# johannes-graeter/limo

Hardware: AMD Instinct MI355X
Metric: keyframe-BA window solves/sec (5 KF, ~2k landmarks) (higher is better)
Workload: dtype f64; 1 GPU; C2: KITTI-00-shaped windows, 5 keyframes x 2000 landmarks, LiDAR depth + ground plane, solveTrimmed schedule {2, trim 5%, <=100 LM iterations}; batch_windows_per_gpu=16384, distinct_windows_per_gpu=4096, observations_per_batch=144288124, depth_observations_per_batch=68405568, parallelism=single, converged=16328

## Files before the change

### limo_amd/csrc/kba_batch_plan.hpp

```cpp
#pragma once
#include <algorithm>
#include <cstdint>
#include <vector>

#include "kba_items.hpp"
#include "kba_pack.hpp"

namespace kba {

struct PlanKernelSizes {
    int (*lean_lds)(int ncol);
    int (*wide_lds)(int nfp, int nc, int n_view);
    int lin_lds;
    int wide_waves;
    int trim_max_sort;
};

struct BatchPlan {
    bool any_fast = false, any_gen = false;
    int plain_tm = 1, plain_wpe = 4, gp_tm = 1, gp_wpe = 3;
    bool pair_ok = false;
    int wide_npw = 0;
    int plain_lds = 0, leangp_lds = 0, wide_lds = 0;
    int max_nc = 0;
    int asm_bytes = 0, solve_bytes = 0, trim_bytes = 0;
    int schur_wave_lds = 0;
    int onelaunch_lds = 0;
};

inline BatchPlan plan_batch(const PackedBatch& P, const PlanKernelSizes& ks) {
    BatchPlan p;
    int t_gen = 1, nfp_gen = 16, nc_gen = kCamSlots, nv_gen = 1, max_nfq = 0, max_nf = 0;
    for (const WinDesc& d : P.win) {
        p.max_nc = std::max(p.max_nc, (int)d.nc);
        if (d.schur_fast) {
            p.any_fast = true;
            max_nfq = std::max(max_nfq, (int)d.nfq);
            max_nf = std::max(max_nf, (int)d.nf);
        } else if (d.n_sblk > 0) {
            p.any_gen = true;
            t_gen = std::max(t_gen, d.nf_pad / 16);
            nfp_gen = std::max(nfp_gen, (int)d.nf_pad);
            nc_gen = std::max(nc_gen, (int)d.nc);
            nv_gen = std::max(nv_gen, (int)d.n_view);
        }
    }
    if (p.any_fast) {
        p.plain_tm = (max_nfq + 16) / 16 <= 1 ? 1 : 2;
        p.plain_wpe = p.plain_tm == 1 ? 4 : 3;
        p.plain_lds = ks.lean_lds(max_nfq + 1);
        p.gp_tm = std::min(3, (max_nf + 16) / 16);
        p.gp_wpe = p.gp_tm == 1 ? 3 : 2;
        p.leangp_lds = ks.lean_lds(max_nf + 1);
        p.pair_ok = p.plain_tm == 2 && p.gp_tm == 3;
    }
    if (p.any_gen) {
        const int tiles = t_gen * (t_gen + 1) / 2, npw = (tiles + ks.wide_waves - 1) / ks.wide_waves;
        p.wide_npw = npw <= 1 ? 1 : npw <= 3 ? 3 : npw <= 6 ? 6 : npw <= 12 ? 12 : -1;
        p.wide_lds = ks.wide_lds(nfp_gen, nc_gen, nv_gen);
    }
    {
        int nc_lds = kCamSlots, nf_lds = 1, nv_lds = 1;
        for (const WinDesc& d : P.win)
            if (d.cam_scr_off < 0) {
                nc_lds = std::max(nc_lds, (int)d.nc);
                nf_lds = std::max(nf_lds, (int)d.nf);
                nv_lds = std::max(nv_lds, (int)d.n_view);
            }
        p.asm_bytes = cam_assemble_scratch(nc_lds, kBlock, nv_lds) * (int)sizeof(double);
        p.solve_bytes = cam_solve_scratch(nc_lds, kBlock, nf_lds) * (int)sizeof(double);
    }
    int max_lm = 1, np2 = 1;
    for (const WinDesc& d : P.win) max_lm = std::max(max_lm, (int)d.n_lm);
    while (np2 < max_lm) np2 <<= 1;
    p.trim_bytes = np2 <= ks.trim_max_sort ? np2 * 12 + max_lm + 16 : 16;
    p.schur_wave_lds = (std::max(p.plain_lds, p.leangp_lds) + 15) / 16 * 16;
    p.onelaunch_lds = std::max(std::max(p.asm_bytes, p.solve_bytes), std::max(p.trim_bytes, ks.lin_lds));
    return p;
}

inline void build_sblk_list(const PackedBatch& P, const std::vector<int32_t>* windows, int span, int span_gp, int owner, std::vector<int32_t>& v,
                            int& n_plain, int& n_fgp) {
    v.clear();
    n_plain = n_fgp = 0;
    const int nw = windows ? (int)windows->size() : P.n_win;
    for (int cls = 0; cls < 3; ++cls) {
        for (int q = 0; q < nw; ++q) {
            const int w = windows ? (*windows)[q] : q;
            const WinDesc& d = P.win[w];
// ... 15 lines not shown
```

### limo_amd/csrc/kba_kernels.hip

```cpp
#include <hip/hip_runtime.h>

#include <type_traits>

#define KBA_SYNC() __syncthreads()
#include "kba_items.hpp"

namespace kba {

__device__ __forceinline__ double wave_sum(double v) {
#pragma unroll
    for (int off = 32; off > 0; off >>= 1) v += __shfl_down(v, off, 64);
    return v;
}
__device__ __forceinline__ double wave_max(double v) {
#pragma unroll
    for (int off = 32; off > 0; off >>= 1) v = fmax(v, __shfl_down(v, off, 64));
    return v;
}

template <int N>
__device__ __forceinline__ void block_sum(const double* vals, double* lds , double* out_global) {
    const int lane = threadIdx.x & 63, wave = threadIdx.x >> 6;
#pragma unroll
    for (int i = 0; i < N; ++i) {
        const double s = wave_sum(vals[i]);
        if (lane == 0) lds[wave * N + i] = s;
    }
    __syncthreads();
    if (threadIdx.x < N) {
        out_global[threadIdx.x] = (lds[threadIdx.x] + lds[N + threadIdx.x]) + (lds[2 * N + threadIdx.x] + lds[3 * N + threadIdx.x]);
    }
}

__device__ __forceinline__ double dpp_mov(double x, int ctrl_sel) {
    int lo = __double2loint(x), hi = __double2hiint(x);
    switch (ctrl_sel) {
        case 0:
            lo = __builtin_amdgcn_update_dpp(0, lo, 0x128, 0xF, 0xF, false);
            hi = __builtin_amdgcn_update_dpp(0, hi, 0x128, 0xF, 0xF, false);
            break;
        case 1:
            lo = __builtin_amdgcn_update_dpp(0, lo, 0x141, 0xF, 0xF, false);
            hi = __builtin_amdgcn_update_dpp(0, hi, 0x141, 0xF, 0xF, false);
            break;
        case 2:
            lo = __builtin_amdgcn_update_dpp(0, lo, 0x4E, 0xF, 0xF, false);
            hi = __builtin_amdgcn_update_dpp(0, hi, 0x4E, 0xF, 0xF, false);
            break;
        default:
            lo = __builtin_amdgcn_update_dpp(0, lo, 0xB1, 0xF, 0xF, false);
            hi = __builtin_amdgcn_update_dpp(0, hi, 0xB1, 0xF, 0xF, false);
            break;
    }
    return __hiloint2double(hi, lo);
}
__device__ __forceinline__ double swap32_add(double a, double b) {
    auto lo = __builtin_amdgcn_permlane32_swap((unsigned)__double2loint(a), (unsigned)__double2loint(b), false, false);
    auto hi = __builtin_amdgcn_permlane32_swap((unsigned)__double2hiint(a), (unsigned)__double2hiint(b), false, false);
    return __hiloint2double((int)hi[0], (int)lo[0]) + __hiloint2double((int)hi[1], (int)lo[1]);
}
__device__ __forceinline__ double swap16_add(double a, double b) {
    auto lo = __builtin_amdgcn_permlane16_swap((unsigned)__double2loint(a), (unsigned)__double2loint(b), false, false);
    auto hi = __builtin_amdgcn_permlane16_swap((unsigned)__double2hiint(a), (unsigned)__double2hiint(b), false, false);
    return __hiloint2double((int)hi[0], (int)lo[0]) + __hiloint2double((int)hi[1], (int)lo[1]);
}
template <int CTRL>
__device__ __forceinline__ double halve_dpp(double a, double b, bool bit) {
    const double keep = bit ? b : a, send = bit ? a : b;
    return keep + dpp_mov(send, CTRL);
}
__device__ __forceinline__ double wave_sum_all(double v) {
    v = swap32_add(v, v);
    v = swap16_add(v, v);
    v += dpp_mov(v, 0);
    v += dpp_mov(v, 1);
    v += dpp_mov(v, 2);
    return v + dpp_mov(v, 3);
}
__device__ __forceinline__ int rs28_index(int lane) {
    const int row = lane >> 4, b3 = (lane >> 3) & 1, b2 = (lane >> 2) & 1, b1 = (lane >> 1) & 1;
    int j;
    if (!b1 && !b2) j = b3 ? 4 : 0;
    else if (!b1 && b2) j = b3 ? 6 : 2;
    else if (b1 && !b2) j = b3 ? 5 : 1;
    else j = b3 ? -1 : 3;
    return (lane & 1) || j < 0 ? -1 : 7 * row + j;
}
__device__ __forceinline__ double wave_reduce_scatter28(const double* v, int lane) {
    double s[14], u[7];
#pragma unroll
    for (int i = 0; i < 14; ++i) s[i] = swap32_add(v[i], v[i + 14]);
#pragma unroll
    for (int i = 0; i < 7; ++i) u[i] = swap16_add(s[i], s[i + 7]);
    const bool b3 = lane & 8, b2 = lane & 4, b1 = lane & 2;
    const double w0 = halve_dpp<0>(u[0], u[4], b3), w1 = halve_dpp<0>(u[1], u[5], b3), w2 = halve_dpp<0>(u[2], u[6], b3);
    const double w3 = u[3] + dpp_mov(u[3], 0);
    const double x0 = halve_dpp<1>(w0, w2, b2), x1 = halve_dpp<1>(w1, w3, b2);
    const double y = halve_dpp<2>(x0, x1, b1);
    return y + dpp_mov(y, 3);
}
__device__ __forceinline__ int rs14_index(int lane) {
    const int half = lane >> 5, rowp = (lane >> 4) & 1, b3 = (lane >> 3) & 1, b2 = (lane >> 2) & 1;
    const int j = b2 ? (b3 ? 3 : 1) : (b3 ? 2 : 0);
    if ((lane & 3) || (j == 3 && rowp)) return -1;
    return 7 * half + (j == 3 ? 3 : j + 4 * rowp);
}
__device__ __forceinline__ double wave_reduce_scatter14(const double* v, int lane) {
    double s[7];
#pragma unroll
    for (int i = 0; i < 7; ++i) s[i] = swap32_add(v[i], v[i + 7]);
    const double u0 = swap16_add(s[0], s[4]), u1 = swap16_add(s[1], s[5]), u2 = swap16_add(s[2], s[6]);
    const double u3 = swap16_add(s[3], s[3]);
    const bool b3 = lane & 8, b2 = lane & 4;
    const double w0 = halve_dpp<0>(u0, u2, b3), w1 = halve_dpp<0>(u1, u3, b3);
    const double x = halve_dpp<1>(w0, w1, b2);
    const double y = x + dpp_mov(x, 2);
    return y + dpp_mov(y, 3);
}
__device__ __forceinline__ void block_sum28(const double* vals, double* lds, double* out_global) {
    const int lane = threadIdx.x & 63, wave = threadIdx.x >> 6;
    const double tot = wave_reduce_scatter28(vals, lane);
    const int idx = rs28_index(lane);
    if (idx >= 0) lds[wave * 28 + idx] = tot;
    __syncthreads();
    if (threadIdx.x < 28) out_global[threadIdx.x] = (lds[threadIdx.x] + lds[28 + threadIdx.x]) + (lds[56 + threadIdx.x] + lds[84 + threadIdx.x]);
}

__device__ __forceinline__ int wl_at(const BatchView& bv, const int32_t* wl, int i) {
    if (bv.counted) return i < wl[-1] ? wl[i] : -1;
    return wl ? wl[i] : i;
}

__global__ void k_solve_init(BatchView bv, SolveConsts c, int max_iter, int select) {
    const int w = blockIdx.x * blockDim.x + threadIdx.x;
    if (w >= bv.n_win) return;
    WinState& s = bv.st[w];
    bool sel = true;
    if (select >= 1) sel = bv.win[w].do_trim != 0;
    if (select == 2) sel = sel && (s.solve_initial_cost - s.solve_final_cost <= 0.0);
    lm_solve_init(s, sel, max_iter, c);
}

__global__ void k_export_active(BatchView bv, int32_t* flags) {
    const int w = blockIdx.x * blockDim.x + threadIdx.x;
    if (w < bv.n_win) flags[w] = bv.st[w].active;
}

__global__ void k_expire(BatchView bv) {
    const int w = blockIdx.x * blockDim.x + threadIdx.x;
    if (w >= bv.n_win) return;
    if (bv.st[w].active) lm_terminate(bv.st[w], LIMO_NO_CONVERGENCE);
}

constexpr int kSchedThreads = 1024;
constexpr int kSchedSlotsPerLane = 4;
constexpr int kSchedMaxSlots = kSchedThreads * kSchedSlotsPerLane;

__global__ void k_sched_advance(BatchView bv, SolveConsts c) {
    const int s = blockIdx.x * blockDim.x + threadIdx.x;
    if (s >= bv.n_slots) return;
    int32_t* cnt = bv.slot_cnt + (int64_t)s * (SL_COUNT + 1);
#pragma unroll
    for (int k = 0; k <= SL_COUNT; ++k) cnt[k] = 0;
    const bool pending = *(volatile int32_t*)bv.sched_ctl < bv.n_win;
    int w = bv.slot_win[s];
    const int w_in = w;
    int kind = 0, n_fin = 0;
    for (int tries = 0; tries < 2; ++tries) {
        if (w < 0) {
            if (!pending) break;
            const int nxt = atomicAdd(bv.sched_ctl, 1);
            if (nxt >= bv.n_win) break;
            w = nxt;
            bv.st[w].phase = PH_IDLE;
        }
        const int r = sched_advance(bv.st[w], bv.win[w], c);
        if (r == 2) {
            ++n_fin;
            w = -1;
            continue;
        }
        kind = r == 1 ? (bv.st[w].phase == PH_TRIM ? 2 : 1) : 0;
        break;
    }
    if (n_fin) atomicAdd(bv.sched_ctl + 1, n_fin);
    if (w != w_in) bv.slot_win[s] = w;
    if (w < 0 || !kind) return;
    const WinDesc& wd = bv.win[w];
    cnt[SL_COUNT] = kind;
    if (kind == 2) {
        cnt[SL_TBLK] = wd.n_blk;
        cnt[SL_TLBLK] = wd.n_lblk;
        cnt[SL_TWIN] = 1;
        return;
    }
    const int gp_groups = (wd.n_sblk - wd.n_sblk_plain + c.schur_span_gp - 1) / c.schur_span_gp;
    const int pl_groups = (wd.n_sblk_plain + c.schur_span - 1) / c.schur_span;
    cnt[SL_LBLK] = wd.n_lblk;
    if (wd.schur_fast) {
        cnt[SL_SPLAIN] = pl_groups;
        cnt[SL_SFGP] = gp_groups;
    } else {
        cnt[SL_SGEN] = pl_groups + gp_groups;
    }
    cnt[SL_WIN] = 1;
}

__global__ __launch_bounds__(kSchedThreads) void k_sched_scan(BatchView bv, int round) {
    __shared__ int wave_tot[16][SL_COUNT];
    const int t = threadIdx.x, lane = t & 63, wave = t >> 6;
    int cnt[kSchedSlotsPerLane][SL_COUNT], tot[SL_COUNT];
#pragma unroll
    for (int k = 0; k < SL_COUNT; ++k) tot[k] = 0;
#pragma unroll
    for (int q = 0; q < kSchedSlotsPerLane; ++q) {
        const int s = t * kSchedSlotsPerLane + q;
#pragma unroll
        for (int k = 0; k < SL_COUNT; ++k) {
            cnt[q][k] = s < bv.n_slots ? bv.slot_cnt[(int64_t)s * (SL_COUNT + 1) + k] : 0;
            tot[k] += cnt[q][k];
        }
    }
    int off[SL_COUNT];
#pragma unroll
    for (int k = 0; k < SL_COUNT; ++k) {
        int x = tot[k];
#pragma unroll
        for (int d = 1; d < 64; d <<= 1) {
            const int y = __shfl_up(x, d, 64);
            if (lane >= d) x += y;
        }
        off[k] = x - tot[k];
        if (lane == 63) wave_tot[wave][k] = x;
    }
    __syncthreads();
    if (t < SL_COUNT) {
        int run = 0;
        for (int q = 0; q < 16; ++q) {
            const int v = wave_tot[q][t];
            wave_tot[q][t] = run;
            run += v;
        }
        bv.sched_lists[bv.sched_off[t]] = run;
    }
    __syncthreads();
#pragma unroll
    for (int q = 0; q < kSchedSlotsPerLane; ++q) {
        const int s = t * kSchedSlotsPerLane + q;
        if (s >= bv.n_slots) continue;
#pragma unroll
        for (int k = 0; k < SL_COUNT; ++k) {
            bv.slot_cnt[(int64_t)s * (SL_COUNT + 1) + k] = wave_tot[wave][k] + off[k];
            off[k] += cnt[q][k];
        }
    }
    if (t == 0) {
        const int done = bv.sched_ctl[1];
        *(volatile int32_t*)(bv.sched_done_host + (round & 3)) = done;
        __threadfence_system();
    }
}

__global__ __launch_bounds__(256) void k_sched_fill(BatchView bv, SolveConsts c) {
    const int s = blockIdx.x * 4 + (threadIdx.x >> 6), lane = threadIdx.x & 63;
    if (s >= bv.n_slots) return;
    const int32_t* off = bv.slot_cnt + (int64_t)s * (SL_COUNT + 1);
    const int kind = off[SL_COUNT];
    if (!kind) return;
    const int w = bv.slot_win[s];
    const WinDesc& wd = bv.win[w];
    auto L = [&](int k) { return bv.sched_lists + bv.sched_off[k] + 1 + off[k]; };
    if (kind == 2) {
        for (int i = lane; i < wd.n_blk; i += 64) L(SL_TBLK)[i] = wd.blk0 + i;
        for (int i = lane; i < wd.n_lblk; i += 64) L(SL_TLBLK)[i] = wd.lblk0 + i;
        if (lane == 0) L(SL_TWIN)[0] = w;
        return;
    }
    for (int i = lane; i < wd.n_lblk; i += 64) L(SL_LBLK)[i] = wd.lblk0 + i;
    const int n_pg = (wd.n_sblk_plain + c.schur_span - 1) / c.schur_span;
    const int n_gg = (wd.n_sblk - wd.n_sblk_plain + c.schur_span_gp - 1) / c.schur_span_gp;
    int32_t* lp = wd.schur_fast ? L(SL_SPLAIN) : L(SL_SGEN);
    int32_t* lg = wd.schur_fast ? L(SL_SFGP) : L(SL_SGEN) + n_pg;
    for (int i = lane; i < n_pg; i += 64) lp[i] = wd.sblk0 + i * c.schur_span;
    for (int i = lane; i < n_gg; i += 64) lg[i] = wd.sblk0 + wd.n_sblk_plain + i * c.schur_span_gp;
    if (lane == 0) L(SL_WIN)[0] = w;
    const WinState& st = bv.st[w];
    if (st.active && st.need_lin && lane < wd.n_view) view_consts_item(bv, wd.view0 + lane);
}

__global__ void k_view_consts(BatchView bv) {
    const int v = blockIdx.x * blockDim.x + threadIdx.x;
    if (v >= bv.TV) return;
    const WinState& st = bv.st[bv.view_win[v]];
    if (!st.active || !st.need_lin) return;
    view_consts_item(bv, v);
}

typedef const double __attribute__((address_space(4))) cdouble;
constexpr int kLinAccl = 13;
constexpr int kLinVlds = 38;
template <bool VLDS>
__device__ __forceinline__ void lin_lm_block(const BatchView& bv, const SolveConsts& c, int b) {
    const int w = bv.lblk_win[b];
    const WinState& st = bv.st[w];
    if (!st.active || !st.need_lin) return;
    const bool want_cost = st.first != 0;
    const WinDesc& wd = bv.win[w];
    const int n_view = wd.n_view;
    const int n = bv.lblk_n[b];
    const int lane = threadIdx.x & 63, wave = threadIdx.x >> 6;
    const bool in_block = (int)threadIdx.x < n;
    const int gl = bv.lblk_lm0[b] + (in_block ? (int)threadIdx.x : n - 1);
    const int state = in_block ? bv.lm_state[gl] : 0;
    LinIn in;
    const bool take_candidate = st.accept != 0;
    const double* lm_src = take_candidate ? bv.lm_c : bv.lm;
    in.p[0] = lm_src[3 * (int64_t)gl];
    in.p[1] = lm_src[3 * (int64_t)gl + 1];
    in.p[2] = lm_src[3 * (int64_t)gl + 2];
    if (take_candidate && in_block) {
        bv.lm[3 * (int64_t)gl] = in.p[0];
        bv.lm[3 * (int64_t)gl + 1] = in.p[1];
        bv.lm[3 * (int64_t)gl + 2] = in.p[2];
    }
    in.w = bv.lm_weight[gl];
    in.sw = sqrt(in.w);
    LmTailIn tail;
    lin_lm_tail_fetch(bv, w, gl, tail);
    const int32_t* slot = bv.lm_slot + gl;
    double* out = bv.lv_part + wd.lvpart_off + (int64_t)(b - wd.lblk0) * n_view * kLinPartial;
    extern __shared__ __attribute__((aligned(16))) double lin_lds[];
    double* const vlds = lin_lds + kLinAccl * kBlock;
    double* const lv_lds = vlds + (VLDS ? n_view * kLinVlds : 0);
    double* const accl = lin_lds + threadIdx.x;
    typedef typename std::conditional<VLDS, const double*, cdouble*>::type VT;
    constexpr int kVStride = VLDS ? kLinVlds : kViewLin;
    VT vc;
    if constexpr (VLDS) {
        const double* src = bv.view_lin + (int64_t)kViewLin * wd.view0;
        for (int i = threadIdx.x; i < n_view * kLinVlds; i += kBlock) vlds[i] = src[(i / kLinVlds) * kViewLin + i % kLinVlds];
        __syncthreads();
        vc = vlds;
    } else {
        vc = (VT)(bv.view_lin + (int64_t)kViewLin * wd.view0);
    }
    const int64_t dump = bv.SO - kObsBlock + threadIdx.x;
#pragma unroll
    for (int i = 0; i < 9; ++i) accl[i * kBlock] = 0.0;
#pragma unroll
    for (int i = 0; i < 3; ++i) accl[(9 + i) * kBlock] = tail.sc[i];
    accl[12 * kBlock] = __hiloint2double(tail.gg, 0);
    auto accum = [&](auto vl, const double* r3, const double* c4) {
        LmAcc a;
#pragma unroll
// ... 1503 lines not shown
```

### limo_amd/csrc/kba_layout.hpp

```cpp
#pragma once
#include <stddef.h>
#include <stdint.h>

#include "../../include/limo_hip.h"

namespace kba {

constexpr int kMaxKf = 20;
constexpr int kMaxViews = 64;
constexpr int kViewLin = 64;
constexpr int kCamSlots = 10;
constexpr int kMaxNc = kMaxKf * kCamSlots;
constexpr int kBlock = 256;
constexpr int kObsPerLane = 4;
constexpr int kObsBlock = kBlock * kObsPerLane;
constexpr int kSchurLm = 16;
constexpr int kSchurLmPerBlock = 64;
constexpr int kSchurSpan = 2, kSchurSpanGp = 1;
constexpr int kMaxRegRows = 1 + (kMaxKf - 1) * 5 + 3 * kMaxKf;

constexpr int kGpRed = 65;
constexpr int kLinPartial = 28;
constexpr int kLinWaves = 4;

// ... 102 lines not shown
    int32_t slab_packed;
};

struct BatchView {
    int32_t n_win, TK, TL, TO, TV, TG, n_blk, n_lblk, n_sblk, Vmax;
    int64_t SO, SL, SG;
    const WinDesc* win;
    WinState* st;
    WinRed* red;
    double *pose, *pdir, *pdist, *lm;
    double *pose_c, *pdir_c, *pdist_c, *lm_c;
    const int32_t* kf_win;
    const int32_t* kf_blk0;
    const int32_t* kf_nblk;
    const int32_t* kf_gp0;
    const int32_t* kf_ngp;
    uint8_t* cmask;
    uint8_t* cpresent;
    const int32_t* cslot;
    const int32_t* lm_win;
    const int32_t* lm_id;
    const double* lm_weight;
    uint8_t* lm_state;
    const int32_t* lm_gp;
    const int32_t* lm_slot;
    const int32_t* view_kf;
    const int32_t* view_win;
    const double* view_cam;
    double* view_lin_c;
    double* view_lin;
    const int32_t* blk_view;
    const int32_t* blk_obs0;
    const int32_t* blk_n;
    const int32_t* obs_lm;
    const float *obs_u, *obs_v, *obs_d;
    const int32_t* lblk_win;
    const int32_t* lblk_lm0;
    const int32_t* lblk_n;
    const int32_t* sblk_win;
    const int32_t* sblk_lm0;
    const int32_t* sblk_n;
    const SchurGroup* sgrp;
    const int32_t* lblk_owner;
    const int32_t* gp_owner;
    double* x_lv;
    double* x_lf;
    double* x_gp;
    double* x_gc;
    double* x_gcc;
    double* x_lb;
    const double* gp_red;
    int32_t gp_red_P, pad_x;
    const int32_t* gp_lm;
    const int32_t* gp_kf;
    const double* gp_w;
    double *gp_r, *gp_F, *gp_E;
    double* gp_cost;
    double* gp_cost_c;
    double *obs_r, *obs_c;
    double *obs_Jp, *obs_Jl;
    const EvalChunk* echunk;
    int64_t SD;
    int32_t n_echunk, pad_e;
    double* lv_part;
    double* lblk_linfail;
    double *lm_V, *lm_g;
    double *lm_scale;
    double* lm_Li;
    double* lblk_part;
    double *Hcc, *gc;
    double *scale_c, *yc, *delta_c;
    double *S_part;
    double *S_red;
    double* cam_scratch;
    double* reg_cost;
    double *trim_rep, *trim_dep;
    int32_t* n_active;
    int32_t* n_active_host;
    int32_t counted;
    int32_t n_slots;
    int32_t* slot_win;
    int32_t* sched_ctl;
    int32_t* slot_cnt;
    int32_t* sched_lists;
    int32_t sched_off[SL_COUNT];
    int32_t* sched_done_host;
};

struct ExchangeLayout {
    int P = 1, n_win = 0, TK = 0;
    size_t n_lv = 0, n_w = 0, n_gp = 0, n_lb = 0, n_S = 0;
    size_t b_lv = 0, b_lf = 0, b_gp = 0, b_gc = 0, b_gcc = 0, b_lb = 0, b_S = 0, b_total = 0;
    size_t c_lv = 0, c_lf = 0, c_gp = 0, c_gc = 0, c_gcc = 0, c_lb = 0, c_S = 0, c_total = 0;
    size_t trim_count = 0;
    size_t spart_count = 1;
#if defined(__HIPCC__)
    __host__ __device__
#endif
    void range(int point, size_t& off, size_t& count) const {
        off = point == 2 ? b_S : point == 4 ? b_gcc : 0;
        const size_t end = point == 1 || point == 4 ? b_S : b_total;
        count = end - off;
    }
};

}
```

### limo_amd/csrc/limo_hip.hip

```cpp
#include <hip/hip_runtime.h>
#include <rccl/rccl.h>

#include <algorithm>
#include <chrono>
#include <cmath>
#include <cstdio>
#include <cstring>
#include <atomic>
#include <memory>
#include <new>
#include <string>
#include <thread>
#include <vector>

#include "kba_kernels.hip"

#include "kba_batch_plan.hpp"
#include "kba_buffers.hpp"
#include "kba_rows.hpp"

using namespace kba;

#include "limo_ctx.hpp"

// ... 545 lines not shown
    }

    void step() override {
        hipStream_t s = ctx->stream;
        if (c.slab_packed) spart_has_packed = true;
        const WorkLists& a = wl[0].cur;
        for (size_t i = 0; i < pv.size(); ++i)
            if (wl[i].cur.n_lblk) {
                hipLaunchKernelGGL(k_lm_damp, dim3(wl[i].cur.n_lblk), dim3(kBlock), 0, s, pv[i], c, wl[i].cur.lblk);
                LAUNCH_CHECK("k_lm_damp");
            }
        {
            EventPair* ep = timed(LIMO_KERNEL_SCHUR);
            for (size_t i = 0; i < pv.size(); ++i) {
                const WorkLists& l = wl[i].cur;
                launch_schur(pv[i], l.sblk, l.n_sblk_plain, l.sblk + l.n_sblk_plain, l.n_sblk_fgp, l.sblk + l.n_sblk_plain + l.n_sblk_fgp,
                             l.n_sblk - l.n_sblk_plain - l.n_sblk_fgp, false, s);
                LAUNCH_CHECK("Schur kernels");
            }
            if (ep) note(hipEventRecord(ep->b, s), "hipEventRecord");
        }
        if (shard_P > 1) {
            if (a.n_win)
                for (size_t i = 0; i < pv.size(); ++i) {
                    hipLaunchKernelGGL(k_shard_reduce, dim3(a.n_win), dim3(kBlock), 0, s, pv[i], a.win, local_shards[i], 1);
                    hipLaunchKernelGGL(k_slab_reduce, dim3(a.n_win, 8), dim3(kBlock), 0, s, pv[i], a.win, shard_P);
                    LAUNCH_CHECK("k_slab_reduce");
                }
            if (assemble_pending) {
                assemble_pending = false;
                exchange(3);
                assemble(it_no - 1);
            } else {
                exchange(2);
            }
        }
        if (a.n_win) hipLaunchKernelGGL(k_cam_solve, dim3(a.n_win), dim3(kBlock), plan.solve_bytes, s, bv, c, a.win);
        LAUNCH_CHECK("k_cam_solve");
        for (size_t i = 0; i < pv.size(); ++i) {
            if (wl[i].cur.n_lblk) {
                hipLaunchKernelGGL(k_backsub, dim3(wl[i].cur.n_lblk), dim3(kBlock), 0, s, pv[i], c, wl[i].cur.lblk);
                LAUNCH_CHECK("k_backsub");
            }
        }
        if (shard_P > 1 && a.n_win)
            for (size_t i = 0; i < pv.size(); ++i) {
                hipLaunchKernelGGL(k_shard_reduce, dim3(a.n_win), dim3(kBlock), 0, s, pv[i], a.win, local_shards[i], 2);
                LAUNCH_CHECK("k_shard_reduce");
            }
        exchange(4);
        if (a.n_win) hipLaunchKernelGGL(k_step_decide, dim3(a.n_win), dim3(64), 0, s, bv, c, a.win);
        LAUNCH_CHECK("k_step_decide");
        hipLaunchKernelGGL(k_accept, dim3(cdiv((int64_t)P.TK + P.TL, 256)), dim3(256), 0, s, bv);
        LAUNCH_CHECK("k_accept");
    }

    void trim() override {
        hipStream_t s = ctx->stream;
        bool any = false;
        for (const WinDesc& d : P.win) any = any || d.do_trim;
        if (!any) return;
        for (size_t i = 0; i < pv.size(); ++i) {
            if (wl[i].full.n_blk) {
                hipLaunchKernelGGL(k_trim_residual, dim3(wl[i].full.n_blk), dim3(kBlock), 0, s, pv[i], d_plane_rep, d_plane_dep, wl[i].full.blk);
                LAUNCH_CHECK("k_trim_residual");
            }
        }
        if (P.TL) {
            for (size_t i = 0; i < pv.size(); ++i) {
                hipLaunchKernelGGL(k_trim_max, dim3(cdiv(P.TL, 256)), dim3(256), 0, s, pv[i], (const double*)d_plane_rep,
                                   (const double*)d_plane_dep, local_shards[i], shard_P);
                LAUNCH_CHECK("k_trim_max");
            }
        }
        exchange_trim();
        hipLaunchKernelGGL(k_trim_select, dim3(P.n_win), dim3(kBlock), plan.trim_bytes, s, bv, c);
        LAUNCH_CHECK("k_trim_select");
    }

    struct StreamGroup {
        hipStream_t stream = nullptr, trim_stream = nullptr;
        bool own_stream = false;
        hipEvent_t sched_ev = nullptr, trim_ev = nullptr, done_ev = nullptr, round_ev[4] = {nullptr, nullptr, nullptr, nullptr};
        int32_t *d_slot_win = nullptr, *d_lists = nullptr, *d_slot_cnt = nullptr;
        int32_t *h_done = nullptr, *d_h_done = nullptr;
        int n_slots = 0;
        int cap[SL_COUNT] = {0};
        int mx[SL_COUNT] = {0};
        BatchView sv;
    };
    std::vector<StreamGroup> groups;
    int stream_groups_built = 0;
    hipEvent_t start_ev = nullptr;

    void stream_teardown() {
        for (StreamGroup& g : groups) {
            if (g.own_stream && g.stream) (void)hipStreamDestroy(g.stream);
            if (g.trim_stream) (void)hipStreamDestroy(g.trim_stream);
            for (hipEvent_t e : {g.sched_ev, g.trim_ev, g.done_ev, g.round_ev[0], g.round_ev[1], g.round_ev[2], g.round_ev[3]})
                if (e) (void)hipEventDestroy(e);
            if (g.h_done) ctx->host_free(g.h_done, 64);
        }
        groups.clear();
        if (start_ev) (void)hipEventDestroy(start_ev);
        start_ev = nullptr;
    }

    int stream_slots() const { return std::min((int)P.n_win, std::max(1024, std::min(kSchedMaxSlots, (int)P.n_win / 4))); }
    int stream_setup(int n_groups) {
        if (stream_groups_built == n_groups) return LIMO_OK;
        (void)hipStreamSynchronize(ctx->stream);
        stream_teardown();
        n_slots = stream_slots();
        int mx[SL_COUNT] = {0};
        for (const WinDesc& d : P.win) {
            const int plg = (d.n_sblk_plain + c.schur_span - 1) / c.schur_span, gpg = (d.n_sblk - d.n_sblk_plain + c.schur_span_gp - 1) / c.schur_span_gp;
            mx[SL_LBLK] = std::max(mx[SL_LBLK], (int)d.n_lblk);
            mx[SL_TBLK] = std::max(mx[SL_TBLK], (int)d.n_blk);
            mx[SL_SPLAIN] = std::max(mx[SL_SPLAIN], d.schur_fast ? plg : 0);
            mx[SL_SFGP] = std::max(mx[SL_SFGP], d.schur_fast ? gpg : 0);
            mx[SL_SGEN] = std::max(mx[SL_SGEN], d.schur_fast ? 0 : plg + gpg);
        }
        mx[SL_WIN] = 1;
        mx[SL_TLBLK] = mx[SL_LBLK];
        mx[SL_TWIN] = 1;
        if (!d_sched_ctl && dmalloc((void**)&d_sched_ctl, sizeof(int32_t) * 8)) return LIMO_ERR_RUNTIME;
        HIP_TRY(ctx, hipEventCreateWithFlags(&start_ev, hipEventDisableTiming));
        groups.resize(n_groups);
        for (int gi = 0; gi < n_groups; ++gi) {
            StreamGroup& g = groups[gi];
            g.n_slots = n_slots / n_groups + (gi < n_slots % n_groups ? 1 : 0);
            g.sv = bv;
            size_t total = 0;
            for (int k = 0; k < SL_COUNT; ++k) {
                g.mx[k] = mx[k];
                g.cap[k] = g.n_slots * mx[k];
                g.sv.sched_off[k] = (int32_t)total;
                total += 1 + (size_t)std::max(1, g.cap[k]);
            }
            if (dmalloc((void**)&g.d_lists, sizeof(int32_t) * total)) return LIMO_ERR_RUNTIME;
            if (dmalloc((void**)&g.d_slot_win, sizeof(int32_t) * std::max(1, g.n_slots))) return LIMO_ERR_RUNTIME;
            if (dmalloc((void**)&g.d_slot_cnt, sizeof(int32_t) * (SL_COUNT + 1) * std::max(1, g.n_slots))) return LIMO_ERR_RUNTIME;
            HIP_TRY(ctx, hipMemsetAsync(g.d_lists, 0, sizeof(int32_t) * total, ctx->stream));
            HIP_TRY(ctx, ctx->host_alloc((void**)&g.h_done, 64));
            HIP_TRY(ctx, hipHostGetDevicePointer((void**)&g.d_h_done, g.h_done, 0));
            for (auto& e : g.round_ev) HIP_TRY(ctx, hipEventCreateWithFlags(&e, hipEventDisableTiming));
            HIP_TRY(ctx, hipEventCreateWithFlags(&g.sched_ev, hipEventDisableTiming));
            HIP_TRY(ctx, hipEventCreateWithFlags(&g.trim_ev, hipEventDisableTiming));
            HIP_TRY(ctx, hipEventCreateWithFlags(&g.done_ev, hipEventDisableTiming));
            HIP_TRY(ctx, hipStreamCreateWithFlags(&g.trim_stream, hipStreamNonBlocking));
            if (gi == 0) {
                g.stream = nullptr;
            } else {
                HIP_TRY(ctx, hipStreamCreateWithFlags(&g.stream, hipStreamNonBlocking));
                g.own_stream = true;
            }
            g.sv.counted = 1;
            g.sv.n_slots = g.n_slots;
            g.sv.slot_win = g.d_slot_win;
            g.sv.sched_ctl = d_sched_ctl;
            g.sv.slot_cnt = g.d_slot_cnt;
            g.sv.sched_lists = g.d_lists;
            g.sv.sched_done_host = g.d_h_done;
            g.sv.n_active_host = nullptr;
        }
        HIP_TRY(ctx, hipStreamSynchronize(ctx->stream));
        stream_groups_built = n_groups;
        return LIMO_OK;
    }

    void enqueue_round(StreamGroup& g, int round, bool time_kernels, int in_flight_max) {
        hipStream_t s = g.stream;
        const BatchView& sv = g.sv;
        int cap[SL_COUNT];
        const int bound = std::max(1, std::min(g.n_slots, in_flight_max));
        for (int k = 0; k < SL_COUNT; ++k) cap[k] = std::min(g.cap[k], bound * g.mx[k]);
        auto L = [&](int k) { return (const int32_t*)(g.d_lists + sv.sched_off[k] + 1); };
        if (round > 0) note(hipStreamWaitEvent(s, g.trim_ev, 0), "wait trim");
        hipLaunchKernelGGL(k_sched_advance, dim3(cdiv(g.n_slots, 256)), dim3(256), 0, s, sv, c);
        hipLaunchKernelGGL(k_sched_scan, dim3(1), dim3(kSchedThreads), 0, s, sv, round);
        hipLaunchKernelGGL(k_sched_fill, dim3(cdiv(g.n_slots, 4)), dim3(256), 0, s, sv, c);
        LAUNCH_CHECK("scheduler kernels");
        note(hipEventRecord(g.sched_ev, s), "record sched");
        note(hipStreamWaitEvent(g.trim_stream, g.sched_ev, 0), "wait sched");
        if (cap[SL_TBLK]) hipLaunchKernelGGL(k_trim_residual, dim3(cap[SL_TBLK]), dim3(kBlock), 0, g.trim_stream, sv, d_plane_rep, d_plane_dep, L(SL_TBLK));
        if (cap[SL_TLBLK]) hipLaunchKernelGGL(k_trim_max, dim3(cap[SL_TLBLK]), dim3(kBlock), 0, g.trim_stream, sv, (const double*)d_plane_rep, (const double*)d_plane_dep, 0, 1);
        hipLaunchKernelGGL(k_trim_select, dim3(cap[SL_TWIN]), dim3(kBlock), plan.trim_bytes, g.trim_stream, sv, c);
        LAUNCH_CHECK("trim kernels");
        note(hipEventRecord(g.trim_ev, g.trim_stream), "record trim");
        {
            EventPair* ep = time_kernels ? timed(LIMO_KERNEL_LINEARIZE, s) : nullptr;
            if (cap[SL_LBLK]) launch_lin_lm(cap[SL_LBLK], s, sv, L(SL_LBLK));
            if (ep) note(hipEventRecord(ep->b, s), "hipEventRecord");
        }
        hipLaunchKernelGGL(k_cam_assemble, dim3(cap[SL_WIN]), dim3(kBlock), plan.asm_bytes, s, sv, c, L(SL_WIN));
        LAUNCH_CHECK("linearisation kernels");
        {
            EventPair* ep = time_kernels ? timed(LIMO_KERNEL_SCHUR, s) : nullptr;
            const bool pair = schur_pair_ok && bound <= kSchurPairBound && cap[SL_SPLAIN] && cap[SL_SFGP];
            launch_schur(sv, L(SL_SPLAIN), cap[SL_SPLAIN], L(SL_SFGP), cap[SL_SFGP], L(SL_SGEN), cap[SL_SGEN], pair, s);
            if (ep) note(hipEventRecord(ep->b, s), "hipEventRecord");
        }
        hipLaunchKernelGGL(k_cam_solve, dim3(cap[SL_WIN]), dim3(kBlock), plan.solve_bytes, s, sv, c, L(SL_WIN));
        if (cap[SL_LBLK]) hipLaunchKernelGGL(k_backsub, dim3(cap[SL_LBLK]), dim3(kBlock), 0, s, sv, c, L(SL_LBLK));
        hipLaunchKernelGGL(k_step_decide, dim3(cap[SL_WIN]), dim3(64), 0, s, sv, c, L(SL_WIN));
        if (cap[SL_LBLK])
            hipLaunchKernelGGL(k_after_step, dim3(cap[SL_LBLK]), dim3(kBlock), 0, s, sv, c, L(SL_LBLK));
        LAUNCH_CHECK("step kernels");
        note(hipEventRecord(g.round_ev[round & 3], s), "record round");
    }

    static constexpr int kWgMaxLblk = 8;
    bool wg_solve_applies() const {
        if (shard_P != 1 || P.evaluate_only || P.n_sblk != 0 || P.n_win < 1) return false;
        if (const char* e = std::getenv("KBA_NO_WG_SOLVE"))
            if (std::atoi(e) != 0) return false;
        for (const WinDesc& d : P.win)
            if (d.n_lblk > kWgMaxLblk) return false;
        return wg_lds_bytes() <= kCamLdsCapBytes;
    }
    int wg_lds_bytes() const { return plan.onelaunch_lds; }
    long long cap_ticks() const { return opts.max_solver_time_sec > 0.0 ? std::max(1ll, (long long)(opts.max_solver_time_sec * 1e8)) : 0ll; }
    void solve_wg() {
        const int lds = wg_lds_bytes();
        note(hipFuncSetAttribute((const void*)k_solve_wg, hipFuncAttributeMaxDynamicSharedMemorySize, lds), "hipFuncSetAttribute(k_solve_wg)");
        hipLaunchKernelGGL(k_solve_wg, dim3(P.n_win), dim3(kBlock), lds, ctx->stream, bv, c, cap_ticks(), d_plane_rep, d_plane_dep);
        LAUNCH_CHECK("k_solve_wg");
    }

    static constexpr int kCoopMaxWg = 256, kCoopMaxWin = 64;
    int32_t* d_coop_bar = nullptr;
    double* d_coop_red = nullptr;
    bool coop_launched = false;
    int coop_G = 0, coop_xcd = 1;
    int coop_lds_bytes() const { return std::max(plan.onelaunch_lds, (kBlock / 64) * plan.schur_wave_lds); }
    bool coop_solve_applies() {
        if (shard_P != 1 || P.evaluate_only || P.n_win < 1) return false;
        if (const char* e = std::getenv("KBA_NO_COOP_SOLVE"))
            if (std::atoi(e) != 0) return false;
        int G = 1;
        for (const WinDesc& d : P.win) {
            if (!d.schur_fast || d.cam_scr_off >= 0 || d.nf_pad * d.nf_pad > kCoopRedStride) return false;
            const int tasks = (d.n_sblk_plain + c.schur_span - 1) / c.schur_span + (d.n_sblk - d.n_sblk_plain + c.schur_span_gp - 1) / c.schur_span_gp;
            G = std::max(G, std::max((int)d.n_lblk, tasks ? 1 + (tasks + kBlock / 64 - 1) / (kBlock / 64) : 1));
        }
        G = std::min(G, 32);
        if (P.n_win > kCoopMaxWg || coop_lds_bytes() > kCamLdsCapBytes) return false;
        const int per8 = ((int)P.n_win + 7) / 8;
        coop_xcd = 8 * per8 > kCoopMaxWg ? 0 : 1;
        G = std::max(1, std::min(G, coop_xcd ? kCoopMaxWg / (8 * per8) : kCoopMaxWg / (int)P.n_win));
        coop_G = G;
        return true;
    }
    bool solve_coop() {
        const int lds = coop_lds_bytes();
        if (!d_coop_bar && dmalloc((void**)&d_coop_bar, sizeof(int32_t) * 8 * P.n_win)) return false;
        if (!d_coop_red && dmalloc((void**)&d_coop_red, sizeof(double) * kCoopRedStride * P.n_win)) return false;
        if (hipFuncSetAttribute((const void*)k_solve_coop, hipFuncAttributeMaxDynamicSharedMemorySize, lds) != hipSuccess) {
            (void)hipGetLastError();
            return false;
        }
        note(hipMemsetAsync(d_coop_bar, 0, sizeof(int32_t) * 8 * P.n_win, ctx->stream), "memset barrier words");
        if (spart_has_packed) {
            note(hipMemsetAsync(bv.S_part, 0, sizeof(double) * (size_t)std::max<int64_t>(1, P.spart_total), ctx->stream), "clear packed Schur slabs");
            spart_has_packed = false;
        }
        h_active[8] = 0;
        CoopParams cp;
        cp.G = coop_G;
        cp.xcd_map = coop_xcd;
        const int coop_grid = coop_xcd ? 8 * coop_G * (((int)P.n_win + 7) / 8) : (int)P.n_win * coop_G;
        cp.vp = plan.plain_tm;
        cp.vg = plan.gp_tm;
        cp.schur_lds = plan.schur_wave_lds / (int)sizeof(double);
        cp.cap_ticks = cap_ticks();
        cp.timeout_ticks = 5000000ll;
        if (const char* e = std::getenv("KBA_COOP_TIMEOUT_MS")) cp.timeout_ticks = std::max(0ll, (long long)(std::atof(e) * 1e5));
        cp.bar = d_coop_bar;
        cp.abort_host = d_h_active + 8;
        cp.plane_rep = d_plane_rep;
        cp.plane_dep = d_plane_dep;
        cp.red = d_coop_red;
        SolveConsts cc = c;
        cc.slab_packed = 0;
        void* args[] = {(void*)&bv, (void*)&cc, (void*)&cp};
        int per_cu = 0, n_cu = 0;
        if (hipOccupancyMaxActiveBlocksPerMultiprocessor(&per_cu, (const void*)k_solve_coop, kBlock, (size_t)lds) != hipSuccess ||
            hipDeviceGetAttribute(&n_cu, hipDeviceAttributeMultiprocessorCount, ctx->device) != hipSuccess || per_cu * n_cu < coop_grid) {
            (void)hipGetLastError();
            return false;
        }
        if (hipLaunchKernel((const void*)k_solve_coop, dim3(coop_grid), dim3(kBlock), args, lds, ctx->stream) != hipSuccess) {
            (void)hipGetLastError();
            return false;
        }
        coop_launched = true;
        return true;
    }

    int solve_streaming() {
        int n_groups = stream_slots() >= 4096 ? 3 : P.n_win >= 512 ? 2 : 1;
        if (const char* e = std::getenv("KBA_GROUPS")) n_groups = std::max(1, std::min(4, std::atoi(e)));
        if (stream_setup(n_groups) != LIMO_OK) return LIMO_ERR_RUNTIME;
        if (c.slab_packed) spart_has_packed = true;
        hipStream_t s0 = ctx->stream;
        groups[0].stream = s0;
        HIP_TRY(ctx, hipMemsetAsync(d_sched_ctl, 0, sizeof(int32_t) * 8, s0));
        for (StreamGroup& g : groups) {
            HIP_TRY(ctx, hipMemsetAsync(g.d_slot_win, 0xFF, sizeof(int32_t) * std::max(1, g.n_slots), s0));
            for (int i = 0; i < 4; ++i) g.h_done[i] = 0;
        }
        HIP_TRY(ctx, hipEventRecord(start_ev, s0));
        for (size_t gi = 1; gi < groups.size(); ++gi) HIP_TRY(ctx, hipStreamWaitEvent(groups[gi].stream, start_ev, 0));
        const bool time_kernels = groups.size() == 1;
        constexpr int kLag = 2;
        static const bool sched_trace = std::getenv("KBA_SCHED_TRACE") != nullptr;
        std::vector<int> done_curve;
        double enq_us = 0.0;
        const auto t_solve0 = std::chrono::steady_clock::now();
        bool finished = false;
        int done_seen = 0;
        for (int round = 0; !finished; ++round) {
            const int in_flight_max = (int)P.n_win - done_seen;
            const auto t_enq0 = std::chrono::steady_clock::now();
            for (StreamGroup& g : groups) enqueue_round(g, round, time_kernels, in_flight_max);
            if (sched_trace) enq_us += std::chrono::duration<double, std::micro>(std::chrono::steady_clock::now() - t_enq0).count();
            if (rc != LIMO_OK) break;
            if (round >= kLag) {
                finished = true;
                for (StreamGroup& g : groups) {
                    note(hipEventSynchronize(g.round_ev[(round - kLag) & 3]), "sync round");
                    if (rc != LIMO_OK) break;
                    const int d = g.h_done[(round - kLag) & 3];
                    if (d < P.n_win) finished = false;
                    done_seen = std::max(done_seen, d);
                }
                if (sched_trace) done_curve.push_back(groups[0].h_done[(round - kLag) & 3]);
            }
            if (round > 200000) {
                rc = LIMO_ERR_RUNTIME;
                ctx->err = "streaming solve did not terminate";
                break;
            }
        }
        if (sched_trace && !done_curve.empty()) {
            const int R = (int)done_curve.size();
            long long occ = 0;
            std::fprintf(stderr, "[kba] streaming solve: %d windows, %d slots, %d groups, %d rounds; in flight at 0,10,..100 %% of the rounds:", (int)P.n_win, n_slots, (int)groups.size(), R);
            for (int r = 0; r < R; ++r) occ += std::min(n_slots, (int)P.n_win - done_curve[r]);
            for (int d = 0; d <= 10; ++d) std::fprintf(stderr, " %d", std::min(n_slots, (int)P.n_win - done_curve[std::min(R - 1, d * R / 10)]));
            std::fprintf(stderr, "; mean occupancy %.3f; host: %.1f us per round inside the enqueue calls, %.1f us per round wall\n", (double)occ / ((double)R * n_slots),
                         enq_us / (R + kLag), std::chrono::duration<double, std::micro>(std::chrono::steady_clock::now() - t_solve0).count() / (R + kLag));
        }
        for (StreamGroup& g : groups) {
            note(hipStreamWaitEvent(g.stream, g.trim_ev, 0), "wait trim");
            if (g.stream != s0) {
                note(hipEventRecord(g.done_ev, g.stream), "record done");
                note(hipStreamWaitEvent(s0, g.done_ev, 0), "wait group");
            }
        }
        return rc;
    }

    int collect_linearize_events() {
        if (ev_used) {
            HIP_TRY(ctx, hipStreamSynchronize(ctx->stream));
            for (size_t i = 0; i < ev_used; ++i) {
                float ms = 0.f;
                HIP_TRY(ctx, hipEventElapsedTime(&ms, ev_pool[i].a, ev_pool[i].b));
                k_ms_acc[ev_pool[i].kernel] += ms;
                k_launches[ev_pool[i].kernel] += 1;
            }
            ev_used = 0;
        }
        return LIMO_OK;
    }
};

extern "C" {

int limo_abi_version(void) {
    return LIMO_ABI_VERSION;
}

int limo_ctx_create(int device, limo_ctx** out) {
    if (!out) return LIMO_ERR_INVALID;
// ... 688 lines not shown
```

Measured before the change: 37620 windows/s.

## Fuse per-block slot scan into scheduler advance and make the scan hierarchical

```diff
diff --git a/limo_amd/csrc/kba_batch_plan.hpp b/limo_amd/csrc/kba_batch_plan.hpp
--- a/limo_amd/csrc/kba_batch_plan.hpp
+++ b/limo_amd/csrc/kba_batch_plan.hpp
@@ -5,6 +5,7 @@
 
 #include "kba_items.hpp"
 #include "kba_pack.hpp"
+#include "kba_stream_plan.hpp"
 
 namespace kba {
 
diff --git a/limo_amd/csrc/kba_kernels.hip b/limo_amd/csrc/kba_kernels.hip
--- a/limo_amd/csrc/kba_kernels.hip
+++ b/limo_amd/csrc/kba_kernels.hip
@@ -4,6 +4,7 @@
 
 #define KBA_SYNC() __syncthreads()
 #include "kba_items.hpp"
+#include "kba_stream_plan.hpp"
 
 namespace kba {
 
@@ -152,109 +153,120 @@
     if (bv.st[w].active) lm_terminate(bv.st[w], LIMO_NO_CONVERGENCE);
 }
 
-constexpr int kSchedThreads = 1024;
-constexpr int kSchedSlotsPerLane = 4;
-constexpr int kSchedMaxSlots = kSchedThreads * kSchedSlotsPerLane;
-
-__global__ void k_sched_advance(BatchView bv, SolveConsts c) {
-    const int s = blockIdx.x * blockDim.x + threadIdx.x;
-    if (s >= bv.n_slots) return;
-    int32_t* cnt = bv.slot_cnt + (int64_t)s * (SL_COUNT + 1);
-#pragma unroll
-    for (int k = 0; k <= SL_COUNT; ++k) cnt[k] = 0;
-    const bool pending = *(volatile int32_t*)bv.sched_ctl < bv.n_win;
-    int w = bv.slot_win[s];
-    const int w_in = w;
-    int kind = 0, n_fin = 0;
-    for (int tries = 0; tries < 2; ++tries) {
-        if (w < 0) {
-            if (!pending) break;
-            const int nxt = atomicAdd(bv.sched_ctl, 1);
-            if (nxt >= bv.n_win) break;
-            w = nxt;
-            bv.st[w].phase = PH_IDLE;
-        }
-        const int r = sched_advance(bv.st[w], bv.win[w], c);
-        if (r == 2) {
-            ++n_fin;
-            w = -1;
-            continue;
-        }
-        kind = r == 1 ? (bv.st[w].phase == PH_TRIM ? 2 : 1) : 0;
-        break;
-    }
-    if (n_fin) atomicAdd(bv.sched_ctl + 1, n_fin);
-    if (w != w_in) bv.slot_win[s] = w;
-    if (w < 0 || !kind) return;
-    const WinDesc& wd = bv.win[w];
-    cnt[SL_COUNT] = kind;
-    if (kind == 2) {
-        cnt[SL_TBLK] = wd.n_blk;
-        cnt[SL_TLBLK] = wd.n_lblk;
-        cnt[SL_TWIN] = 1;
-        return;
-    }
-    const int gp_groups = (wd.n_sblk - wd.n_sblk_plain + c.schur_span_gp - 1) / c.schur_span_gp;
-    const int pl_groups = (wd.n_sblk_plain + c.schur_span - 1) / c.schur_span;
-    cnt[SL_LBLK] = wd.n_lblk;
-    if (wd.schur_fast) {
-        cnt[SL_SPLAIN] = pl_groups;
-        cnt[SL_SFGP] = gp_groups;
-    } else {
-        cnt[SL_SGEN] = pl_groups + gp_groups;
-    }
-    cnt[SL_WIN] = 1;
-}
-
-__global__ __launch_bounds__(kSchedThreads) void k_sched_scan(BatchView bv, int round) {
-    __shared__ int wave_tot[16][SL_COUNT];
-    const int t = threadIdx.x, lane = t & 63, wave = t >> 6;
-    int cnt[kSchedSlotsPerLane][SL_COUNT], tot[SL_COUNT];
-#pragma unroll
-    for (int k = 0; k < SL_COUNT; ++k) tot[k] = 0;
-#pragma unroll
-    for (int q = 0; q < kSchedSlotsPerLane; ++q) {
-        const int s = t * kSchedSlotsPerLane + q;
-#pragma unroll
-        for (int k = 0; k < SL_COUNT; ++k) {
-            cnt[q][k] = s < bv.n_slots ? bv.slot_cnt[(int64_t)s * (SL_COUNT + 1) + k] : 0;
-            tot[k] += cnt[q][k];
-        }
-    }
-    int off[SL_COUNT];
+__device__ __forceinline__ void sched_block_scan(int (&v)[SL_COUNT], int (&tot)[SL_COUNT], int (*lds)[SL_COUNT]) {
+    constexpr int kWaves = kSchedBlock / 64;
+    const int lane = threadIdx.x & 63, wave = threadIdx.x >> 6;
 #pragma unroll
     for (int k = 0; k < SL_COUNT; ++k) {
-        int x = tot[k];
+        int x = v[k];
 #pragma unroll
         for (int d = 1; d < 64; d <<= 1) {
             const int y = __shfl_up(x, d, 64);
             if (lane >= d) x += y;
         }
-        off[k] = x - tot[k];
-        if (lane == 63) wave_tot[wave][k] = x;
+        v[k] = x - v[k];
+        if (lane == 63) lds[wave][k] = x;
     }
     __syncthreads();
-    if (t < SL_COUNT) {
-        int run = 0;
-        for (int q = 0; q < 16; ++q) {
-            const int v = wave_tot[q][t];
-            wave_tot[q][t] = run;
-            run += v;
-        }
-        bv.sched_lists[bv.sched_off[t]] = run;
+#pragma unroll
+    for (int k = 0; k < SL_COUNT; ++k) {
+        int pre = 0, all = 0;
+#pragma unroll
+        for (int q = 0; q < kWaves; ++q) {
+            const int w = lds[q][k];
+            pre += q < wave ? w : 0;
+            all += w;
+        }
+        v[k] += pre;
+        tot[k] = all;
     }
     __syncthreads();
-#pragma unroll
-    for (int q = 0; q < kSchedSlotsPerLane; ++q) {
-        const int s = t * kSchedSlotsPerLane + q;
-        if (s >= bv.n_slots) continue;
+}
+
+__global__ __launch_bounds__(kSchedBlock) void k_sched_advance(BatchView bv, SolveConsts c) {
+    __shared__ int wave_tot[kSchedBlock / 64][SL_COUNT];
+    const int s = blockIdx.x * kSchedBlock + threadIdx.x;
+    int cnt[SL_COUNT], tot[SL_COUNT];
+#pragma unroll
+    for (int k = 0; k < SL_COUNT; ++k) cnt[k] = 0;
+    int kind = 0;
+    if (s < bv.n_slots) {
+        const bool pending = *(volatile int32_t*)bv.sched_ctl < bv.n_win;
+        int w = bv.slot_win[s];
+        const int w_in = w;
+        int n_fin = 0;
+        for (int tries = 0; tries < 2; ++tries) {
+            if (w < 0) {
+                if (!pending) break;
+                const int nxt = atomicAdd(bv.sched_ctl, 1);
+                if (nxt >= bv.n_win) break;
+                w = nxt;
+                bv.st[w].phase = PH_IDLE;
+            }
+            const int r = sched_advance(bv.st[w], bv.win[w], c);
+            if (r == 2) {
+                ++n_fin;
+                w = -1;
+                continue;
+            }
+            kind = r == 1 ? (bv.st[w].phase == PH_TRIM ? 2 : 1) : 0;
+            break;
+        }
+        if (n_fin) atomicAdd(bv.sched_ctl + 1, n_fin);
+        if (w != w_in) bv.slot_win[s] = w;
+        if (w < 0) kind = 0;
+        if (kind == 2) {
+            const WinDesc& wd = bv.win[w];
+            cnt[SL_TBLK] = wd.n_blk;
+            cnt[SL_TLBLK] = wd.n_lblk;
+            cnt[SL_TWIN] = 1;
+        } else if (kind == 1) {
+            const WinDesc& wd = bv.win[w];
+            const int gp_groups = (wd.n_sblk - wd.n_sblk_plain + c.schur_span_gp - 1) / c.schur_span_gp;
+            const int pl_groups = (wd.n_sblk_plain + c.schur_span - 1) / c.schur_span;
+            cnt[SL_LBLK] = wd.n_lblk;
+            if (wd.schur_fast) {
+                cnt[SL_SPLAIN] = pl_groups;
+                cnt[SL_SFGP] = gp_groups;
+            } else {
+                cnt[SL_SGEN] = pl_groups + gp_groups;
+            }
+            cnt[SL_WIN] = 1;
+        }
+    }
+    sched_block_scan(cnt, tot, wave_tot);
+    if (s < bv.n_slots) {
+#pragma unroll
+        for (int k = 0; k < SL_COUNT; ++k) bv.slot_cnt[sched_cnt_index(s, k)] = cnt[k];
+        bv.slot_cnt[sched_cnt_index(s, SL_COUNT)] = kind;
+    }
+    if (threadIdx.x == 0) {
+#pragma unroll
+        for (int k = 0; k < SL_COUNT; ++k) bv.sched_blk[sched_blk_index(blockIdx.x, k)] = tot[k];
+    }
+}
+
+__global__ __launch_bounds__(kSchedBlock) void k_sched_scan(BatchView bv, int round) {
+    __shared__ int wave_tot[kSchedBlock / 64][SL_COUNT];
+    const int t = threadIdx.x, n_blocks = sched_blocks(bv.n_slots);
+    int carry[SL_COUNT];
+#pragma unroll
+    for (int k = 0; k < SL_COUNT; ++k) carry[k] = 0;
+    for (int b0 = 0; b0 < n_blocks; b0 += kSchedBlock) {
+        const int b = b0 + t;
+        int v[SL_COUNT], tot[SL_COUNT];
+#pragma unroll
+        for (int k = 0; k < SL_COUNT; ++k) v[k] = b < n_blocks ? bv.sched_blk[sched_blk_index(b, k)] : 0;
+        sched_block_scan(v, tot, wave_tot);
 #pragma unroll
         for (int k = 0; k < SL_COUNT; ++k) {
-            bv.slot_cnt[(int64_t)s * (SL_COUNT + 1) + k] = wave_tot[wave][k] + off[k];
-            off[k] += cnt[q][k];
+            if (b < n_blocks) bv.sched_blk[sched_blk_index(b, k)] = carry[k] + v[k];
+            carry[k] += tot[k];
         }
     }
     if (t == 0) {
+#pragma unroll
+        for (int k = 0; k < SL_COUNT; ++k) bv.sched_lists[bv.sched_off[k]] = carry[k];
         const int done = bv.sched_ctl[1];
         *(volatile int32_t*)(bv.sched_done_host + (round & 3)) = done;
         __threadfence_system();
@@ -264,12 +276,11 @@
 __global__ __launch_bounds__(256) void k_sched_fill(BatchView bv, SolveConsts c) {
     const int s = blockIdx.x * 4 + (threadIdx.x >> 6), lane = threadIdx.x & 63;
     if (s >= bv.n_slots) return;
-    const int32_t* off = bv.slot_cnt + (int64_t)s * (SL_COUNT + 1);
-    const int kind = off[SL_COUNT];
+    const int kind = bv.slot_cnt[sched_cnt_index(s, SL_COUNT)];
     if (!kind) return;
     const int w = bv.slot_win[s];
     const WinDesc& wd = bv.win[w];
-    auto L = [&](int k) { return bv.sched_lists + bv.sched_off[k] + 1 + off[k]; };
+    auto L = [&](int k) { return bv.sched_lists + bv.sched_off[k] + 1 + sched_slot_offset(bv.slot_cnt, bv.sched_blk, s, k); };
     if (kind == 2) {
         for (int i = lane; i < wd.n_blk; i += 64) L(SL_TBLK)[i] = wd.blk0 + i;
         for (int i = lane; i < wd.n_lblk; i += 64) L(SL_TLBLK)[i] = wd.lblk0 + i;
diff --git a/limo_amd/csrc/kba_layout.hpp b/limo_amd/csrc/kba_layout.hpp
--- a/limo_amd/csrc/kba_layout.hpp
+++ b/limo_amd/csrc/kba_layout.hpp
@@ -208,6 +208,7 @@
     int32_t* slot_win;
     int32_t* sched_ctl;
     int32_t* slot_cnt;
+    int32_t* sched_blk;
     int32_t* sched_lists;
     int32_t sched_off[SL_COUNT];
     int32_t* sched_done_host;
diff --git a/limo_amd/csrc/kba_stream_plan.hpp b/limo_amd/csrc/kba_stream_plan.hpp
--- /dev/null
+++ b/limo_amd/csrc/kba_stream_plan.hpp
@@ -0,0 +1,59 @@
+#pragma once
+#include <stdint.h>
+
+#include "kba_layout.hpp"
+#include "kba_math.hpp"
+
+namespace kba {
+
+constexpr int kSchedBlock = 256;
+
+KBA_HD int sched_blocks(int n_slots) { return (n_slots + kSchedBlock - 1) / kSchedBlock; }
+KBA_HD int sched_block_of(int s) { return s / kSchedBlock; }
+KBA_HD int64_t sched_cnt_index(int s, int k) { return (int64_t)s * (SL_COUNT + 1) + k; }
+KBA_HD int64_t sched_blk_index(int b, int k) { return (int64_t)b * SL_COUNT + k; }
+KBA_HD int sched_slot_offset(const int32_t* slot_cnt, const int32_t* blk, int s, int k) {
+    return blk[sched_blk_index(sched_block_of(s), k)] + slot_cnt[sched_cnt_index(s, k)];
+}
+
+inline void sched_scan_block(int32_t* slot_cnt, int32_t* blk, int n_slots, int b) {
+    int run[SL_COUNT] = {0};
+    const int s1 = n_slots < (b + 1) * kSchedBlock ? n_slots : (b + 1) * kSchedBlock;
+    for (int s = b * kSchedBlock; s < s1; ++s)
+        for (int k = 0; k < SL_COUNT; ++k) {
+            const int v = slot_cnt[sched_cnt_index(s, k)];
+            slot_cnt[sched_cnt_index(s, k)] = run[k];
+            run[k] += v;
+        }
+    for (int k = 0; k < SL_COUNT; ++k) blk[sched_blk_index(b, k)] = run[k];
+}
+inline void sched_scan_blocks(int32_t* blk, int n_blocks, int32_t* len) {
+    for (int k = 0; k < SL_COUNT; ++k) {
+        int run = 0;
+        for (int b = 0; b < n_blocks; ++b) {
+            const int v = blk[sched_blk_index(b, k)];
+            blk[sched_blk_index(b, k)] = run;
+            run += v;
+        }
+        len[k] = run;
+    }
+}
+
+struct StreamPlan {
+    int slots, groups;
+};
+constexpr int kStreamMaxGroups = 4;
+
+constexpr int kStreamMaxSlots = 4096;
+inline int stream_default_slots(int n_win) { return n_win < kStreamMaxSlots ? n_win : kStreamMaxSlots; }
+inline StreamPlan plan_stream(int n_win, int slots_override, int groups_override) {
+    StreamPlan p;
+    n_win = n_win > 1 ? n_win : 1;
+    p.slots = slots_override > 0 ? (slots_override < n_win ? slots_override : n_win) : stream_default_slots(n_win);
+    p.groups = p.slots >= 4096 ? 3 : n_win >= 512 ? 2 : 1;
+    if (groups_override > 0) p.groups = groups_override < kStreamMaxGroups ? groups_override : kStreamMaxGroups;
+    if (p.groups > p.slots) p.groups = p.slots;
+    return p;
+}
+
+}
diff --git a/limo_amd/csrc/limo_hip.hip b/limo_amd/csrc/limo_hip.hip
--- a/limo_amd/csrc/limo_hip.hip
+++ b/limo_amd/csrc/limo_hip.hip
@@ -651,7 +651,7 @@
         hipStream_t stream = nullptr, trim_stream = nullptr;
         bool own_stream = false;
         hipEvent_t sched_ev = nullptr, trim_ev = nullptr, done_ev = nullptr, round_ev[4] = {nullptr, nullptr, nullptr, nullptr};
-        int32_t *d_slot_win = nullptr, *d_lists = nullptr, *d_slot_cnt = nullptr;
+        int32_t *d_slot_win = nullptr, *d_lists = nullptr, *d_slot_cnt = nullptr, *d_sched_blk = nullptr;
         int32_t *h_done = nullptr, *d_h_done = nullptr;
         int n_slots = 0;
         int cap[SL_COUNT] = {0};
@@ -659,7 +659,7 @@
         BatchView sv;
     };
     std::vector<StreamGroup> groups;
-    int stream_groups_built = 0;
+    int stream_groups_built = 0, stream_slots_built = 0;
     hipEvent_t start_ev = nullptr;
 
     void stream_teardown() {
@@ -675,12 +675,11 @@
         start_ev = nullptr;
     }
 
-    int stream_slots() const { return std::min((int)P.n_win, std::max(1024, std::min(kSchedMaxSlots, (int)P.n_win / 4))); }
-    int stream_setup(int n_groups) {
-        if (stream_groups_built == n_groups) return LIMO_OK;
+    int stream_setup(int n_groups, int slots) {
+        if (stream_groups_built == n_groups && stream_slots_built == slots) return LIMO_OK;
         (void)hipStreamSynchronize(ctx->stream);
         stream_teardown();
-        n_slots = stream_slots();
+        n_slots = slots;
         int mx[SL_COUNT] = {0};
         for (const WinDesc& d : P.win) {
             const int plg = (d.n_sblk_plain + c.schur_span - 1) / c.schur_span, gpg = (d.n_sblk - d.n_sblk_plain + c.schur_span_gp - 1) / c.schur_span_gp;
@@ -710,6 +709,7 @@
             if (dmalloc((void**)&g.d_lists, sizeof(int32_t) * total)) return LIMO_ERR_RUNTIME;
             if (dmalloc((void**)&g.d_slot_win, sizeof(int32_t) * std::max(1, g.n_slots))) return LIMO_ERR_RUNTIME;
             if (dmalloc((void**)&g.d_slot_cnt, sizeof(int32_t) * (SL_COUNT + 1) * std::max(1, g.n_slots))) return LIMO_ERR_RUNTIME;
+            if (dmalloc((void**)&g.d_sched_blk, sizeof(int32_t) * SL_COUNT * std::max(1, sched_blocks(g.n_slots)))) return LIMO_ERR_RUNTIME;
             HIP_TRY(ctx, hipMemsetAsync(g.d_lists, 0, sizeof(int32_t) * total, ctx->stream));
             HIP_TRY(ctx, ctx->host_alloc((void**)&g.h_done, 64));
             HIP_TRY(ctx, hipHostGetDevicePointer((void**)&g.d_h_done, g.h_done, 0));
@@ -729,12 +729,14 @@
             g.sv.slot_win = g.d_slot_win;
             g.sv.sched_ctl = d_sched_ctl;
             g.sv.slot_cnt = g.d_slot_cnt;
+            g.sv.sched_blk = g.d_sched_blk;
             g.sv.sched_lists = g.d_lists;
             g.sv.sched_done_host = g.d_h_done;
             g.sv.n_active_host = nullptr;
         }
         HIP_TRY(ctx, hipStreamSynchronize(ctx->stream));
         stream_groups_built = n_groups;
+        stream_slots_built = slots;
         return LIMO_OK;
     }
 
@@ -746,8 +748,8 @@
         for (int k = 0; k < SL_COUNT; ++k) cap[k] = std::min(g.cap[k], bound * g.mx[k]);
         auto L = [&](int k) { return (const int32_t*)(g.d_lists + sv.sched_off[k] + 1); };
         if (round > 0) note(hipStreamWaitEvent(s, g.trim_ev, 0), "wait trim");
-        hipLaunchKernelGGL(k_sched_advance, dim3(cdiv(g.n_slots, 256)), dim3(256), 0, s, sv, c);
-        hipLaunchKernelGGL(k_sched_scan, dim3(1), dim3(kSchedThreads), 0, s, sv, round);
+        hipLaunchKernelGGL(k_sched_advance, dim3(sched_blocks(g.n_slots)), dim3(kSchedBlock), 0, s, sv, c);
+        hipLaunchKernelGGL(k_sched_scan, dim3(1), dim3(kSchedBlock), 0, s, sv, round);
         hipLaunchKernelGGL(k_sched_fill, dim3(cdiv(g.n_slots, 4)), dim3(256), 0, s, sv, c);
         LAUNCH_CHECK("scheduler kernels");
         note(hipEventRecord(g.sched_ev, s), "record sched");
@@ -868,9 +870,9 @@
     }
 
     int solve_streaming() {
-        int n_groups = stream_slots() >= 4096 ? 3 : P.n_win >= 512 ? 2 : 1;
-        if (const char* e = std::getenv("KBA_GROUPS")) n_groups = std::max(1, std::min(4, std::atoi(e)));
-        if (stream_setup(n_groups) != LIMO_OK) return LIMO_ERR_RUNTIME;
+        const char *e_slots = std::getenv("KBA_SLOTS"), *e_groups = std::getenv("KBA_GROUPS");
+        const StreamPlan sp = plan_stream((int)P.n_win, e_slots ? std::max(1, std::atoi(e_slots)) : 0, e_groups ? std::max(1, std::atoi(e_groups)) : 0);
+        if (stream_setup(sp.groups, sp.slots) != LIMO_OK) return LIMO_ERR_RUNTIME;
         if (c.slab_packed) spart_has_packed = true;
         hipStream_t s0 = ctx->stream;
         groups[0].stream = s0;
```

Measured after the change: 37620 windows/s, median of 2. Within noise of the previous version (+0.0%).
